# cloneofsimo/paint-with-words-sd

Hardware: NVIDIA H100
Metric: unet_steps_per_sec_512sq_cfg (higher is better)
Workload: dtype f16

## Files before the change

paint_with_words_sd_b200/csrc/attn_tc.cuh:

```cuda
#pragma once
#include "mma_sm90.cuh"
#include "pww_common.cuh"
#include "xattn_core.cuh"

namespace pww {
namespace fa {

constexpr int kThreads = core::kThreads;
constexpr int kBM = core::kBM;
constexpr int kBN = 64;

template <int D>
struct Cfg {
  using T_ = core::Tile<D>;
  static constexpr uint32_t KVBYTES = kBN * T_::LD * 2;
  static constexpr uint32_t OFF_KV = T_::QBYTES;
  static constexpr uint32_t SMEM = T_::QBYTES + 2 * 2 * KVBYTES;
  static_assert(SMEM <= 232448, "shared memory budget");
};

template <typename E>
struct Params {
  const E* q;
  const E* k;
  const E* v;
  E* out;
  int B, H, N;
  int64_t bs, rs;
  int64_t o_bs, o_rs;
  float scale;
};

template <int D, typename E>
constexpr int kMinBlocks = (D == 80 && std::is_same_v<E, __nv_bfloat16>) ? 1 : 0;

template <int D, typename E>
__global__ void __launch_bounds__(kThreads, kMinBlocks<D, E>) attn_fwd_kernel(const Params<E> p) {
  using C = core::Tile<D>;
  using CF = Cfg<D>;
  extern __shared__ __align__(128) unsigned char smem[];
  const uint32_t smem0 = ptx::smem_u32(smem);
  const int warp = threadIdx.x >> 5, lane = threadIdx.x & 31;
  const int qtiles = (p.N + kBM - 1) / kBM;
  const int bh = blockIdx.x / qtiles, qt = blockIdx.x - bh * qtiles;
  const int b = bh / p.H, h = bh - b * p.H;
  const int row_base = qt * kBM;
  const E* qb = p.q + (int64_t)b * p.bs + h * D;
  const E* kb = p.k + (int64_t)b * p.bs + h * D;
  const E* vb = p.v + (int64_t)b * p.bs + h * D;
  const int ntiles = (p.N + kBN - 1) / kBN;
  auto issue_kv = [&](int j) {
    const uint32_t st = smem0 + CF::OFF_KV + (j & 1) * 2 * CF::KVBYTES;
    const int rows = p.N - j * kBN < kBN ? p.N - j * kBN : kBN;
    core::load_rows<D>(st, kb + (int64_t)j * kBN * p.rs, p.rs, kBN, rows);
    core::load_rows<D>(st + CF::KVBYTES, vb + (int64_t)j * kBN * p.rs, p.rs, kBN, rows);
    ptx::cp_async_commit();
  };
  {
    const int rows = p.N - row_base < kBM ? p.N - row_base : kBM;
    core::load_rows<D>(smem0, qb + (int64_t)row_base * p.rs, p.rs, kBM, rows);
  }
  issue_kv(0);
  uint32_t qa[C::KS][4];
  float o[C::NT][4], m0, m1, l0, l1;
  core::warp_online_begin<D>(o, m0, m1, l0, l1);
  const float sl2 = p.scale * 1.4426950408889634f;
  const uint32_t qs = smem0 + (uint32_t)(warp * 16 * C::LD) * 2u;
#pragma unroll 1
  for (int jt = 0; jt < ntiles; ++jt) {
    if (jt + 1 < ntiles) {
      issue_kv(jt + 1);
      ptx::cp_async_wait<1>();
    } else {
      ptx::cp_async_wait<0>();
    }
    __syncthreads();
    if (jt == 0) {
#pragma unroll
      for (int kk = 0; kk < C::KS; ++kk)
        ptx::ldsm_x4(qs + (uint32_t)((lane & 15) * C::LD + kk * 16 + (lane >> 4) * 8) * 2u, qa[kk][0], qa[kk][1], qa[kk][2], qa[kk][3]);
    }
    const uint32_t ks = smem0 + CF::OFF_KV + (jt & 1) * 2 * CF::KVBYTES, vs = ks + CF::KVBYTES;
    float s[kBN / 8][4];
#pragma unroll
    for (int j = 0; j < kBN / 8; ++j) s[j][0] = s[j][1] = s[j][2] = s[j][3] = 0.f;
#pragma unroll
    for (int kk = 0; kk < C::KS; ++kk) {
#pragma unroll
      for (int jp = 0; jp < kBN / 16; ++jp) {
        const int t = 16 * jp + (lane & 7) + ((lane >> 4) << 3), d = kk * 16 + ((lane >> 3) & 1) * 8;
        uint32_t b0, b1, b2, b3;
        ptx::ldsm_x4(ks + (uint32_t)(t * C::LD + d) * 2u, b0, b1, b2, b3);
        ptx::mma16816<E>(s[2 * jp], qa[kk], b0, b1);
        ptx::mma16816<E>(s[2 * jp + 1], qa[kk], b2, b3);
      }
    }
    core::warp_online_chunk<D, E>(s, p.N - jt * kBN, sl2, vs, lane, o, m0, m1, l0, l1);
    __syncthreads();
  }
  core::warp_online_end<D>(o, l0, l1);
  core::warp_store<D>(o, smem + warp * 16 * C::LD * 2, lane, p.out + (int64_t)b * p.o_bs + h * D, p.o_rs,
                      row_base + warp * 16, p.N);
}

template <int D, typename E>
cudaError_t launch(const void* q, const void* k, const void* v, void* out, int B, int H, int N, int64_t bs, int64_t rs,
                   int64_t o_bs, int64_t o_rs, float scale, cudaStream_t s) {
  using CF = Cfg<D>;
  Params<E> p;
  p.q = (const E*)q; p.k = (const E*)k; p.v = (const E*)v; p.out = (E*)out;
  p.B = B; p.H = H; p.N = N; p.bs = bs; p.rs = rs; p.o_bs = o_bs; p.o_rs = o_rs; p.scale = scale;
  const cudaError_t e = allow_dynamic_smem<attn_fwd_kernel<D, E>>(CF::SMEM);
  if (e != cudaSuccess) return e;
  const long long grid = (long long)B * H * ((N + kBM - 1) / kBM);
  if (grid > 0x7fffffffLL) return cudaErrorInvalidConfiguration;
  attn_fwd_kernel<D, E><<<(unsigned)grid, kThreads, CF::SMEM, s>>>(p);
  return cudaGetLastError();
}

}
}
```

paint_with_words_sd_b200/csrc/pww_abi.cu:

```cuda
#include <stdio.h>
#include <string.h>

#include "pww_common.cuh"
#include "xattn_tc.cuh"
#include "xattn_fused2.cuh"
#include "attn_tc.cuh"
#include "unet_ops.cuh"
#include "sampler_step.cuh"
#include "control_inject.cuh"
#include "control_combine.cuh"
#include "adapter_residual.cuh"
#include <stdlib.h>
#include <algorithm>
#include <type_traits>

namespace {

thread_local char g_last_cuda_error[640] = "";

int cuda_fail(cudaError_t e);

bool aligned16(const void* p) { return (reinterpret_cast<uintptr_t>(p) & 15u) == 0; }

bool supported_head_dim(int D) { return D == 40 || D == 64 || D == 80 || D == 160; }

int check_common(const void* q, const void* k, int B, int H, int N, int T, int D, int64_t q_bs, int64_t q_rs,
                 int64_t k_bs, int64_t k_rs) {
  if (!q || !k || B <= 0 || H <= 0 || N <= 0 || T <= 0 || D <= 0) return PWW_ERR_BAD_ARG;
  if (!aligned16(q) || !aligned16(k)) return PWW_ERR_BAD_ARG;
  if ((q_bs | q_rs | k_bs | k_rs) & 7) return PWW_ERR_BAD_ARG;
  if (q_rs < (int64_t)H * D || k_rs < (int64_t)H * D) return PWW_ERR_BAD_ARG;
  if (!supported_head_dim(D) || !pww::core::supported_keys(T)) return PWW_ERR_UNSUPPORTED;
  return PWW_OK;
}

template <int D_, int KC_>
struct Shape {
  static constexpr int D = D_, KC = KC_;
};
template <int D, typename F>
cudaError_t with_chunks(int T, F&& f) {
  switch (pww::core::chunks_of(T)) {
    case 1: return f(Shape<D, 1>{});
    case 2: return f(Shape<D, 2>{});
    case 3: return f(Shape<D, 3>{});
  }
  return cudaErrorInvalidValue;
}
template <typename F>
cudaError_t with_shape(int D, int T, F&& f) {
  switch (D) {
    case 40: return with_chunks<40>(T, f);
    case 64: return with_chunks<64>(T, f);
    case 80: return with_chunks<80>(T, f);
    case 160: return with_chunks<160>(T, f);
  }
  return cudaErrorInvalidValue;
}

template <int lo, int hi, typename F>
void with_int(int v, F&& f) {
  if constexpr (lo < hi)
    if (v != lo) return with_int<lo + 1, hi>(v, f);
  f(std::integral_constant<int, lo>{});
}

size_t align_up(size_t x, size_t a) { return (x + a - 1) / a * a; }

constexpr int kStatSlotsPerImage = 2048;

int cuda_fail(cudaError_t e) {
  snprintf(g_last_cuda_error, sizeof(g_last_cuda_error), "%s: %s ", cudaGetErrorName(e), cudaGetErrorString(e));
  return PWW_ERR_CUDA;
}

template <typename E>
pww::XattnParams<E> xattn_params(const void* q, const void* k, const void* v, void* out, int B, int H, int N, int T, int D,
                                 int64_t q_bs, int64_t q_rs, int64_t k_bs, int64_t k_rs, int64_t o_bs, int64_t o_rs) {
  pww::XattnParams<E> p;
  memset(&p, 0, sizeof(p));
  p.q = (const E*)q; p.k = (const E*)k; p.v = (const E*)v; p.out = (E*)out;
  p.B = B; p.H = H; p.N = N; p.T = T; p.D = D;
  p.q_bs = q_bs; p.q_rs = q_rs; p.k_bs = k_bs; p.k_rs = k_rs; p.o_bs = o_bs; p.o_rs = o_rs;
  return p;
}

template <typename E>
pww::XattnParams<E> images(const pww::XattnParams<E>& p, int b0, int n) {
  pww::XattnParams<E> c = p;
  c.B = n;
  c.q += (int64_t)b0 * p.q_bs;
  c.k += (int64_t)b0 * p.k_bs;
  if (c.v) c.v += (int64_t)b0 * p.k_bs;
  if (c.out) c.out += (int64_t)b0 * p.o_bs;
  if (c.wmap_index) c.wmap_index += b0;
  if (c.stat_kind) c.stat_kind += b0;
  if (c.stats) c.stats += b0;
  if (c.stats_out) c.stats_out += b0;
  if (c.g_sigma) c.g_sigma += (int64_t)b0 * p.g_stride;
  return c;
}

}

extern "C" {

int pww_version(void) { return 300; }

const char* pww_status_str(int status) {
  switch (status) {
    case PWW_OK: return "ok";
    case PWW_ERR_BAD_ARG: return "bad argument (null/misaligned pointer, non-positive size or stride not a multiple of 8)";
    case PWW_ERR_UNSUPPORTED: return "unsupported shape or dtype (head dim must be 40/64/80/160, T <= 80, 154 or 231)";
    case PWW_ERR_CUDA: return "CUDA error (see pww_last_cuda_error)";
    case PWW_ERR_WORKSPACE: return "workspace too small (see pww_xattn_workspace_bytes)";
    default: return "unknown status";
  }
}

const char* pww_last_cuda_error(void) { return g_last_cuda_error; }

int pww_device_supported(void) {
  int dev = 0, major = 0;
  cudaError_t e = cudaGetDevice(&dev);
  if (e != cudaSuccess) return cuda_fail(e);
  e = cudaDeviceGetAttribute(&major, cudaDevAttrComputeCapabilityMajor, dev);
  if (e != cudaSuccess) return cuda_fail(e);
  return major == 9 ? 1 : 0;
}

size_t pww_xattn_workspace_bytes(int B, int H, int N, int T, int D) {
  (void)T; (void)D;
  if (B <= 0 || H <= 0 || N <= 0) return 0;
  return align_up((size_t)B * sizeof(unsigned int), 256) +
         (size_t)B * kStatSlotsPerImage * sizeof(pww::StatPartial);
}

}

namespace {

template <typename E>
int xattn_stats(const void* q, const void* k, int B, int H, int N, int T, int D, int64_t q_batch_stride,
                int64_t q_row_stride, int64_t k_batch_stride, int64_t k_row_stride, int stat, const int32_t* kinds,
                bool per_image, const int32_t* wmap_index, float* stats, void* workspace, size_t workspace_bytes,
                void* stream) {
  int rc = check_common(q, k, B, H, N, T, D, q_batch_stride, q_row_stride, k_batch_stride, k_row_stride);
  if (rc) return rc;
  if (!stats || !workspace) return PWW_ERR_BAD_ARG;
  if (per_image ? !kinds : (stat != PWW_STAT_MAX && stat != PWW_STAT_STD)) return PWW_ERR_BAD_ARG;
  if (workspace_bytes < pww_xattn_workspace_bytes(B, H, N, T, D)) return PWW_ERR_WORKSPACE;
  if (pww::num_sms() > kStatSlotsPerImage) return PWW_ERR_WORKSPACE;
  pww::XattnParams<E> p = xattn_params<E>(q, k, nullptr, nullptr, B, H, N, T, D, q_batch_stride, q_row_stride,
                                          k_batch_stride, k_row_stride, 0, 0);
  p.wmap_index = wmap_index; p.stat = stat; p.stat_kind = per_image ? kinds : nullptr; p.stats_out = stats;
  p.counters = (unsigned int*)workspace;
  p.partials = (pww::StatPartial*)((char*)workspace + align_up((size_t)B * sizeof(unsigned int), 256));
  for (int b0 = 0; b0 < B; b0 += pww::tc::kMaxBatch) {
    const pww::XattnParams<E> c = images(p, b0, std::min(B - b0, pww::tc::kMaxBatch));
    const cudaError_t e =
        with_shape(D, T, [&](auto k) { return pww::tc::launch_stats<k.D, k.KC>(c, (cudaStream_t)stream); });
    if (e != cudaSuccess) return cuda_fail(e);
  }
  return PWW_OK;
}

template <typename E>
int xattn_fwd(const void* q, const void* k, const void* v, void* out, int B, int H, int N, int T, int D,
              int64_t q_batch_stride, int64_t q_row_stride, int64_t k_batch_stride, int64_t k_row_stride,
              int64_t o_batch_stride, int64_t o_row_stride, const float* wmap, int64_t wmap_batch_stride,
              const int32_t* wmap_index, const float* stats, const float* g_sigma, int64_t g_stride, float scale,
              void* stream) {
  int rc = check_common(q, k, B, H, N, T, D, q_batch_stride, q_row_stride, k_batch_stride, k_row_stride);
  if (rc) return rc;
  if (!v || !out || !aligned16(v) || !aligned16(out)) return PWW_ERR_BAD_ARG;
  if ((o_batch_stride | o_row_stride) & 7 || o_row_stride < (int64_t)H * D) return PWW_ERR_BAD_ARG;
  if (wmap && (!stats || !g_sigma)) return PWW_ERR_BAD_ARG;
  pww::XattnParams<E> p = xattn_params<E>(q, k, v, out, B, H, N, T, D, q_batch_stride, q_row_stride, k_batch_stride,
                                          k_row_stride, o_batch_stride, o_row_stride);
  p.wmap = wmap; p.wmap_bs = wmap_batch_stride; p.wmap_index = wmap ? wmap_index : nullptr;
  p.stats = stats; p.g_sigma = g_sigma; p.g_stride = g_stride; p.scale = scale;
  for (int b0 = 0; b0 < B; b0 += pww::tc::kMaxBatch) {
    pww::XattnParams<E> c = images(p, b0, std::min(B - b0, pww::tc::kMaxBatch));
    if (wmap && !wmap_index) c.wmap += (int64_t)b0 * wmap_batch_stride;
    const cudaError_t e =
        with_shape(D, T, [&](auto k) { return pww::tc::launch_fwd<k.D, k.KC>(c, (cudaStream_t)stream); });
    if (e != cudaSuccess) return cuda_fail(e);
  }
  return PWW_OK;
}

template <typename E>
int xattn_fused(const void* q, const void* k, const void* v, void* out, int B, int H, int N, int T, int D,
                int64_t q_batch_stride, int64_t q_row_stride, int64_t k_batch_stride, int64_t k_row_stride,
                int64_t o_batch_stride, int64_t o_row_stride, const void* mpack, int64_t mpack_batch_stride, int Bw,
                const int8_t* cidx, const int32_t* wmap_index, int stat, const int32_t* kinds, bool per_image,
                const float* g_sigma, float scale, float* stats, void* workspace, size_t workspace_bytes,
                void* stream, const pww::fx::FxRecord* rec = nullptr) {
  int rc = check_common(q, k, B, H, N, T, D, q_batch_stride, q_row_stride, k_batch_stride, k_row_stride);
  if (rc) return rc;
  if (!v || !out || !aligned16(v) || !aligned16(out)) return PWW_ERR_BAD_ARG;
  if ((o_batch_stride | o_row_stride) & 7 || o_row_stride < (int64_t)H * D || o_batch_stride <= 0) return PWW_ERR_BAD_ARG;
  if (rec && (!rec->ridx || !rec->rec_index || !rec->rec_acc || !aligned16(rec->rec_acc) ||
              rec->rec_bs < (int64_t)H * N * pww::core::kRegions))
    return PWW_ERR_BAD_ARG;
  if (mpack) {
    if (!cidx || !g_sigma || !workspace || Bw <= 0 || !aligned16(mpack)) return PWW_ERR_BAD_ARG;
    if ((mpack_batch_stride & 7) || mpack_batch_stride < (int64_t)N * pww::fx::kMW) return PWW_ERR_BAD_ARG;
    if (per_image ? !kinds : (stat != PWW_STAT_MAX && stat != PWW_STAT_STD)) return PWW_ERR_BAD_ARG;
    if (workspace_bytes < pww_xattn_fused_workspace_bytes()) return PWW_ERR_WORKSPACE;
  }
  pww::XattnParams<E> p = xattn_params<E>(q, k, v, out, B, H, N, T, D, q_batch_stride, q_row_stride, k_batch_stride,
                                          k_row_stride, o_batch_stride, o_row_stride);
  p.g_sigma = g_sigma; p.g_stride = per_image ? 1 : 0; p.scale = scale; p.stat = stat;
  p.stat_kind = per_image ? kinds : nullptr; p.stats_out = stats;
  p.wmap_index = mpack ? wmap_index : nullptr;
  p.counters = (unsigned int*)workspace;
  p.partials = workspace ? (pww::StatPartial*)((char*)workspace + 512) : nullptr;
  int chunk = pww::fx::kMaxBatch;
  const int tiles = pww::ceil_div(N, pww::core::kBM);
  const int hg = pww::ceil_div(H, D == 40 ? pww::fx::Cfg2<40>::G : (D == 64 ? pww::fx::Cfg2<64>::G : 1));
  while (chunk > 1) {
    const int cb = B < chunk ? B : chunk;
    if (pww::fx::fused2_fits(cb, hg, tiles, pww::fx::fused_grid(cb * hg * tiles))) break;
    chunk >>= 1;
  }
  for (int b0 = 0; b0 < B; b0 += chunk) {
    pww::XattnParams<E> c = images(p, b0, std::min(B - b0, chunk));
    const void* mp = mpack;
    const int8_t* ci = cidx;
    if (mpack && !wmap_index) {
      mp = (const __half*)mpack + (int64_t)b0 * mpack_batch_stride;
      ci = cidx + (int64_t)b0 * pww::core::kTP * pww::core::chunks_of(T);
    }
    c.wmap = (const float*)mp;
    pww::fx::FxRecord r;
    if (rec) {
      r = *rec;
      r.rec_index += b0;
    }
    const cudaError_t e = with_shape(D, T, [&](auto k) {
      return pww::fx::launch_fused2<k.D, k.KC>(c, mp, mpack_batch_stride, ci, (cudaStream_t)stream, rec ? &r : nullptr);
    });
    if (e == cudaErrorInvalidConfiguration) return PWW_ERR_UNSUPPORTED;
    if (e != cudaSuccess) return cuda_fail(e);
  }
  return PWW_OK;
}

template <typename E>
int groupnorm_nhwc(const void* x, const void* add, int64_t add_batch_stride, const void* gamma, const void* beta, void* y,
                   int B, int HW, int C, int G, float eps, int silu, void* workspace, size_t workspace_bytes,
                   void* stream) {
  if (!x || !gamma || !beta || !y || !workspace || B <= 0 || HW <= 0 || C <= 0 || G <= 0) return PWW_ERR_BAD_ARG;
  if (!aligned16(x) || !aligned16(y) || !aligned16(gamma) || !aligned16(beta) || (add && !aligned16(add)))
    return PWW_ERR_BAD_ARG;
  if ((C & 7) || (C % G) || G > 64 || (C >> 3) > 1024) return PWW_ERR_UNSUPPORTED;
  if (add && ((add_batch_stride & 7) || add_batch_stride < C)) return PWW_ERR_BAD_ARG;
  if (workspace_bytes < pww_groupnorm_workspace_bytes(B, HW, G)) return PWW_ERR_WORKSPACE;
  const pww::uops::GnSplit sp = pww::uops::gn_split(HW, C, G);
  pww::uops::GnParams<E> p;
  p.x = (const E*)x; p.add = (const E*)add; p.add_bs = add_batch_stride; p.gamma = (const E*)gamma; p.beta = (const E*)beta;
  p.y = (E*)y;
  p.partial = (float2*)workspace;
  p.HW = HW; p.C = C; p.G = G; p.eps = eps; p.silu = silu;
  p.sv = sp.sv; p.chunks = sp.chunks; p.rows_per_chunk = sp.rows_per_chunk;
  cudaStream_t s = (cudaStream_t)stream;
  const size_t smem1 = (64 + (size_t)2 * sp.rpp * sp.sv * 8) * sizeof(float);
  if (smem1 > 48 * 1024) {
    const cudaError_t e = pww::allow_dynamic_smem<pww::uops::gn_stats_kernel<E>>(64 * 1024 + 256);
    if (e != cudaSuccess) return cuda_fail(e);
  }
  pww::uops::gn_stats_kernel<E><<<dim3(sp.chunks, sp.slices, B), sp.threads, smem1, s>>>(p);
  int rows = 4;
  while (rows > 1 && (long long)B * sp.slices * pww::ceil_div(HW, sp.rpp * rows) < 2 * pww::num_sms()) rows >>= 1;
  cudaLaunchAttribute pdl;
  pdl.id = cudaLaunchAttributeProgrammaticStreamSerialization;
  pdl.val.programmaticStreamSerializationAllowed = 1;
  cudaLaunchConfig_t cfg = {};
  cfg.gridDim = dim3(pww::ceil_div(HW, sp.rpp * rows), sp.slices, B);
  cfg.blockDim = dim3(sp.threads);
  cfg.stream = s;
  cfg.attrs = &pdl;
  cfg.numAttrs = 1;
  cudaError_t e = cudaLaunchKernelEx(&cfg, pww::uops::gn_apply_kernel<E>, p, sp.rpp * rows);
  if (e == cudaSuccess) e = cudaGetLastError();
  return e == cudaSuccess ? PWW_OK : cuda_fail(e);
}

template <typename E>
int geglu(const void* in, void* out, int64_t M, int I, void* stream) {
  if (!in || !out || M <= 0 || I <= 0 || !aligned16(in) || !aligned16(out)) return PWW_ERR_BAD_ARG;
  if (I & 7) return PWW_ERR_UNSUPPORTED;
  const long long total = (long long)M * (I >> 3);
  long long blocks = (total + 255) / 256;
  const long long cap = (long long)pww::num_sms() * 16;
  if (blocks > cap) blocks = cap;
  pww::uops::geglu_kernel<E><<<(int)blocks, 256, 0, (cudaStream_t)stream>>>((const E*)in, (E*)out, M, I);
  cudaError_t e = cudaGetLastError();
  return e == cudaSuccess ? PWW_OK : cuda_fail(e);
}

template <typename E>
int add_layernorm(const void* x, const void* res, const void* gamma, const void* beta, void* sum_out, void* y, int64_t M,
                  int C, float eps, void* stream) {
  if (!x || !gamma || !beta || !y || M <= 0 || C <= 0) return PWW_ERR_BAD_ARG;
  if (!aligned16(x) || !aligned16(y) || !aligned16(gamma) || !aligned16(beta) || (res && !aligned16(res)) ||
      (sum_out && !aligned16(sum_out)))
    return PWW_ERR_BAD_ARG;
  if ((C & 7) || C > 2048) return PWW_ERR_UNSUPPORTED;
  const int warps = 8;
  const unsigned grid = (unsigned)((M + warps - 1) / warps);
  with_int<1, 8>(((C >> 3) + 31) / 32, [&](auto vpl) {
    pww::uops::add_layernorm_kernel<E, vpl><<<grid, warps * 32, 0, (cudaStream_t)stream>>>(
        (const E*)x, (const E*)res, (const E*)gamma, (const E*)beta, (E*)sum_out, (E*)y, M, C, eps);
  });
  cudaError_t e = cudaGetLastError();
  return e == cudaSuccess ? PWW_OK : cuda_fail(e);
}

template <typename E>
int resnet_residual(const void* a, const void* h, const float* bias, void* out, int64_t rows, int C, void* stream) {
  if (!a || !h || !bias || !out || rows <= 0 || C <= 0 || (C & 7)) return PWW_ERR_BAD_ARG;
  if (!aligned16(a) || !aligned16(h) || !aligned16(bias) || !aligned16(out)) return PWW_ERR_BAD_ARG;
  const long long total = (long long)rows * (C >> 3);
  long long blocks = (total + 255) / 256;
  const long long cap = (long long)pww::num_sms() * 16;
  if (blocks > cap) blocks = cap;
  pww::uops::resnet_residual_kernel<E><<<(int)blocks, 256, 0, (cudaStream_t)stream>>>(
      (const E*)a, (const E*)h, bias, (E*)out, total, C >> 3);
  cudaError_t e = cudaGetLastError();
  return e == cudaSuccess ? PWW_OK : cuda_fail(e);
}

template <typename E>
int adapter_residual(const void* a, const void* b, const float* bias, const void* feat, void* out, int rows,
                     int64_t pixels, int C, int feat_rows, void* stream) {
  if (!a || !b || !out || rows <= 0 || pixels <= 0 || C <= 0 || (C & 7)) return PWW_ERR_BAD_ARG;
  if (feat_rows < 0 || feat_rows > rows || (feat_rows > 0 && !feat)) return PWW_ERR_BAD_ARG;
  if (!aligned16(a) || !aligned16(b) || !aligned16(out) || (bias && !aligned16(bias)) || (feat && !aligned16(feat)))
    return PWW_ERR_BAD_ARG;
  const long long per_row = (long long)pixels * (C >> 3);
  const cudaError_t e = pww::adp::launch<E>(a, b, bias, feat, out, (long long)rows * per_row,
                                            (long long)feat_rows * per_row, C >> 3, (long long)pww::num_sms() * 16,
                                            (cudaStream_t)stream);
  return e == cudaSuccess ? PWW_OK : cuda_fail(e);
}

template <typename E>
int attn_fwd(const void* q,const void* k, const void* v, void* out, int B, int H, int N, int D, int64_t qkv_batch_stride,
             int64_t qkv_row_stride, int64_t o_batch_stride, int64_t o_row_stride, float scale, void* stream) {
  if (!q || !k || !v || !out || B <= 0 || H <= 0 || N <= 0 || D <= 0) return PWW_ERR_BAD_ARG;
  if (!aligned16(q) || !aligned16(k) || !aligned16(v) || !aligned16(out)) return PWW_ERR_BAD_ARG;
  if ((qkv_batch_stride | qkv_row_stride | o_batch_stride | o_row_stride) & 7) return PWW_ERR_BAD_ARG;
  if (qkv_row_stride < (int64_t)H * D || o_row_stride < (int64_t)H * D) return PWW_ERR_BAD_ARG;
  if (!supported_head_dim(D)) return PWW_ERR_UNSUPPORTED;
  const cudaError_t e = with_shape(D, 1, [&](auto sh) {
    return pww::fa::launch<sh.D, E>(q, k, v, out, B, H, N, qkv_batch_stride, qkv_row_stride, o_batch_stride,
                                    o_row_stride, scale, (cudaStream_t)stream);
  });
  return e == cudaSuccess ? PWW_OK : cuda_fail(e);
}

template <typename E>
int control_inject(int n, void* const* dst, const void* const* res, const int64_t* elems_per_image, int rows,
                   const float* scales, void* stream) {
  if (n < 1 || n > pww::ctl::kMaxLevels || rows < 1 || !dst || !res || !elems_per_image) return PWW_ERR_BAD_ARG;
  pww::ctl::InjectArgs a;
  a.off[0] = 0;
  for (int k = 0; k < n; ++k) {
    const int64_t e = elems_per_image[k];
    if (e <= 0 || (e % pww::ctl::kVec) != 0) return PWW_ERR_BAD_ARG;
    if (!dst[k] || !res[k] || !aligned16(dst[k]) || !aligned16(res[k])) return PWW_ERR_BAD_ARG;
    a.dst[k] = dst[k];
    a.res[k] = res[k];
    a.vec_per_image[k] = e / pww::ctl::kVec;
    a.off[k + 1] = a.off[k] + (int64_t)rows * a.vec_per_image[k];
  }
  for (int k = n; k < pww::ctl::kMaxLevels; ++k) {
    a.dst[k] = nullptr;
    a.res[k] = nullptr;
    a.vec_per_image[k] = 0;
    a.off[k + 1] = a.off[n];
  }
  a.scales = scales;
  a.n = n;
  a.rows = rows;
  const cudaError_t e = pww::ctl::launch_inject<E>(a, (int64_t)pww::num_sms() * 8, (cudaStream_t)stream);
  return e == cudaSuccess ? PWW_OK : cuda_fail(e);
}

template <typename E>
int control_combine(int units, int n, void* const* out, const void* const* res, const int64_t* elems_per_image,
                    int rows, const float* scales, void* stream) {
  if (units < 1 || units > pww::ctl::kMaxUnits || n < 1 || n > pww::ctl::kMaxLevels || rows < 1 || !out || !res ||
      !elems_per_image || !scales)
    return PWW_ERR_BAD_ARG;
  pww::ctl::CombineArgs a = {};
  for (int k = 0; k < n; ++k) {
    const int64_t e = elems_per_image[k];
    if (e <= 0 || (e % pww::ctl::kVec) != 0) return PWW_ERR_BAD_ARG;
    if (!out[k] || !aligned16(out[k])) return PWW_ERR_BAD_ARG;
    a.out[k] = out[k];
    a.vec_per_image[k] = e / pww::ctl::kVec;
    a.off[k + 1] = a.off[k] + (int64_t)rows * a.vec_per_image[k];
  }
  for (int i = 0; i < units * n; ++i) {
    if (!res[i] || !aligned16(res[i])) return PWW_ERR_BAD_ARG;
    a.res[i] = res[i];
  }
  for (int k = n; k < pww::ctl::kMaxLevels; ++k) a.off[k + 1] = a.off[n];
  a.scales = scales;
  a.units = units;
  a.n = n;
  a.rows = rows;
  const cudaError_t e = pww::ctl::launch_combine<E>(a, (int64_t)pww::num_sms() * 8, (cudaStream_t)stream);
  return e == cudaSuccess ? PWW_OK : cuda_fail(e);
}

}

extern "C" {

int pww_xattn_stats_f16(const void* q, const void* k, int B, int H, int N, int T, int D, int64_t q_batch_stride,
    int64_t q_row_stride, int64_t k_batch_stride, int64_t k_row_stride, int stat, const int32_t* wmap_index,
    float* stats, void* workspace, size_t workspace_bytes, void* stream) {
  return xattn_stats<__half>(
      q, k, B, H, N, T, D, q_batch_stride, q_row_stride, k_batch_stride, k_row_stride, stat, nullptr, false,
      wmap_index, stats, workspace, workspace_bytes, stream);
}
int pww_xattn_stats_bf16(const void* q, const void* k, int B, int H, int N, int T, int D, int64_t q_batch_stride,
    int64_t q_row_stride, int64_t k_batch_stride, int64_t k_row_stride, int stat, const int32_t* wmap_index,
    float* stats, void* workspace, size_t workspace_bytes, void* stream) {
  return xattn_stats<__nv_bfloat16>(
      q, k, B, H, N, T, D, q_batch_stride, q_row_stride, k_batch_stride, k_row_stride, stat, nullptr, false,
      wmap_index, stats, workspace, workspace_bytes, stream);
}

int pww_xattn_stats_multi_f16(const void* q, const void* k, int B, int H, int N, int T, int D, int64_t q_batch_stride,
    int64_t q_row_stride, int64_t k_batch_stride, int64_t k_row_stride, const int32_t* stat, const int32_t* wmap_index,
    float* stats, void* workspace, size_t workspace_bytes, void* stream) {
  return xattn_stats<__half>(
      q, k, B, H, N, T, D, q_batch_stride, q_row_stride, k_batch_stride, k_row_stride, PWW_STAT_MAX, stat, true,
      wmap_index, stats, workspace, workspace_bytes, stream);
}
int pww_xattn_stats_multi_bf16(const void* q, const void* k, int B, int H, int N, int T, int D, int64_t q_batch_stride,
    int64_t q_row_stride, int64_t k_batch_stride, int64_t k_row_stride, const int32_t* stat, const int32_t* wmap_index,
    float* stats, void* workspace, size_t workspace_bytes, void* stream) {
  return xattn_stats<__nv_bfloat16>(
      q, k, B, H, N, T, D, q_batch_stride, q_row_stride, k_batch_stride, k_row_stride, PWW_STAT_MAX, stat, true,
      wmap_index, stats, workspace, workspace_bytes, stream);
}

int pww_xattn_fwd_f16(const void* q, const void* k, const void* v, void* out, int B, int H, int N, int T, int D,
    int64_t q_batch_stride, int64_t q_row_stride, int64_t k_batch_stride, int64_t k_row_stride, int64_t o_batch_stride,
    int64_t o_row_stride, const float* wmap, int64_t wmap_batch_stride, const int32_t* wmap_index, const float* stats,
    const float* g_sigma, float scale, void* stream) {
  return xattn_fwd<__half>(q, k, v, out, B, H, N, T, D, q_batch_stride, q_row_stride, k_batch_stride, k_row_stride,
      o_batch_stride, o_row_stride, wmap, wmap_batch_stride, wmap_index, stats, g_sigma, 0, scale, stream);
}
int pww_xattn_fwd_bf16(const void* q, const void* k, const void* v, void* out, int B, int H, int N, int T, int D,
    int64_t q_batch_stride, int64_t q_row_stride, int64_t k_batch_stride, int64_t k_row_stride, int64_t o_batch_stride,
    int64_t o_row_stride, const float* wmap, int64_t wmap_batch_stride, const int32_t* wmap_index, const float* stats,
    const float* g_sigma, float scale, void* stream) {
  return xattn_fwd<__nv_bfloat16>(
      q, k, v, out, B, H, N, T, D, q_batch_stride, q_row_stride, k_batch_stride, k_row_stride,
      o_batch_stride, o_row_stride, wmap, wmap_batch_stride, wmap_index, stats, g_sigma, 0, scale, stream);
}

int pww_xattn_fwd_multi_f16(const void* q, const void* k, const void* v, void* out, int B, int H, int N, int T, int D,
    int64_t q_batch_stride, int64_t q_row_stride, int64_t k_batch_stride, int64_t k_row_stride, int64_t o_batch_stride,
    int64_t o_row_stride, const float* wmap, int64_t wmap_batch_stride, const int32_t* wmap_index, const float* stats,
    const float* g_sigma, float scale, void* stream) {
  return xattn_fwd<__half>(q, k, v, out, B, H, N, T, D, q_batch_stride, q_row_stride, k_batch_stride, k_row_stride,
      o_batch_stride, o_row_stride, wmap, wmap_batch_stride, wmap_index, stats, g_sigma, 1, scale, stream);
}
int pww_xattn_fwd_multi_bf16(const void* q, const void* k, const void* v, void* out, int B, int H, int N, int T, int D,
    int64_t q_batch_stride, int64_t q_row_stride, int64_t k_batch_stride, int64_t k_row_stride, int64_t o_batch_stride,
    int64_t o_row_stride, const float* wmap, int64_t wmap_batch_stride, const int32_t* wmap_index, const float* stats,
    const float* g_sigma, float scale, void* stream) {
  return xattn_fwd<__nv_bfloat16>(
      q, k, v, out, B, H, N, T, D, q_batch_stride, q_row_stride, k_batch_stride, k_row_stride,
      o_batch_stride, o_row_stride, wmap, wmap_batch_stride, wmap_index, stats, g_sigma, 1, scale, stream);
}

size_t pww_xattn_fused_workspace_bytes(void) { return pww::fx::fused_workspace_bytes(); }

int pww_xattn_fused_f16(const void* q, const void* k, const void* v, void* out, int B, int H, int N, int T, int D,
    int64_t q_batch_stride, int64_t q_row_stride, int64_t k_batch_stride, int64_t k_row_stride, int64_t o_batch_stride,
    int64_t o_row_stride, const void* mpack, int64_t mpack_batch_stride, int Bw, const int8_t* cidx,
    const int32_t* wmap_index, int stat, const float* g_sigma, float scale, float* stats, void* workspace,
    size_t workspace_bytes, void* stream) {
  return xattn_fused<__half>(q, k, v, out, B, H, N, T, D, q_batch_stride, q_row_stride, k_batch_stride, k_row_stride,
      o_batch_stride, o_row_stride, mpack, mpack_batch_stride, Bw, cidx, wmap_index, stat, nullptr, false,
      g_sigma, scale, stats, workspace, workspace_bytes, stream);
}
int pww_xattn_fused_bf16(const void* q, const void* k, const void* v, void* out, int B, int H, int N, int T, int D,
    int64_t q_batch_stride, int64_t q_row_stride, int64_t k_batch_stride, int64_t k_row_stride, int64_t o_batch_stride,
    int64_t o_row_stride, const void* mpack, int64_t mpack_batch_stride, int Bw, const int8_t* cidx,
    const int32_t* wmap_index, int stat, const float* g_sigma, float scale, float* stats, void* workspace,
    size_t workspace_bytes, void* stream) {
  return xattn_fused<__nv_bfloat16>(
      q, k, v, out, B, H, N, T, D, q_batch_stride, q_row_stride, k_batch_stride, k_row_stride,
      o_batch_stride, o_row_stride, mpack, mpack_batch_stride, Bw, cidx, wmap_index, stat, nullptr, false,
      g_sigma, scale, stats, workspace, workspace_bytes, stream);
}

int pww_xattn_fused_multi_f16(const void* q, const void* k, const void* v, void* out, int B, int H, int N, int T, int D,
    int64_t q_batch_stride, int64_t q_row_stride, int64_t k_batch_stride, int64_t k_row_stride, int64_t o_batch_stride,
    int64_t o_row_stride, const void* mpack, int64_t mpack_batch_stride, int Bw, const int8_t* cidx,
    const int32_t* wmap_index, const int32_t* stat, const float* g_sigma, float scale, float* stats, void* workspace,
    size_t workspace_bytes, void* stream) {
  return xattn_fused<__half>(q, k, v, out, B, H, N, T, D, q_batch_stride, q_row_stride, k_batch_stride, k_row_stride,
      o_batch_stride, o_row_stride, mpack, mpack_batch_stride, Bw, cidx, wmap_index, PWW_STAT_MAX, stat, true,
      g_sigma, scale, stats, workspace, workspace_bytes, stream);
}
int pww_xattn_fused_multi_bf16(const void* q, const void* k, const void* v, void* out, int B, int H, int N, int T, int D,
    int64_t q_batch_stride, int64_t q_row_stride, int64_t k_batch_stride, int64_t k_row_stride, int64_t o_batch_stride,
    int64_t o_row_stride, const void* mpack, int64_t mpack_batch_stride, int Bw, const int8_t* cidx,
    const int32_t* wmap_index, const int32_t* stat, const float* g_sigma, float scale, float* stats, void* workspace,
    size_t workspace_bytes, void* stream) {
  return xattn_fused<__nv_bfloat16>(
      q, k, v, out, B, H, N, T, D, q_batch_stride, q_row_stride, k_batch_stride, k_row_stride,
      o_batch_stride, o_row_stride, mpack, mpack_batch_stride, Bw, cidx, wmap_index, PWW_STAT_MAX, stat, true,
      g_sigma, scale, stats, workspace, workspace_bytes, stream);
}

int pww_xattn_fused_rec_f16(const void* q, const void* k, const void* v, void* out, int B, int H, int N, int T, int D,
    int64_t q_batch_stride, int64_t q_row_stride, int64_t k_batch_stride, int64_t k_row_stride, int64_t o_batch_stride,
    int64_t o_row_stride, const void* mpack, int64_t mpack_batch_stride, int Bw, const int8_t* cidx,
    const int32_t* wmap_index, const int32_t* stat, const float* g_sigma, float scale, float* stats, void* workspace,
    size_t workspace_bytes, void* stream, const int8_t* ridx, const int32_t* rec_index, float* rec_acc,
    int64_t rec_batch_stride) {
  const pww::fx::FxRecord rec = {ridx, rec_index, rec_acc, rec_batch_stride};
  return xattn_fused<__half>(q, k, v, out, B, H, N, T, D, q_batch_stride, q_row_stride, k_batch_stride, k_row_stride,
      o_batch_stride, o_row_stride, mpack, mpack_batch_stride, Bw, cidx, wmap_index, PWW_STAT_MAX, stat, true,
      g_sigma, scale, stats, workspace, workspace_bytes, stream, &rec);
}
int pww_xattn_fused_rec_bf16(const void* q, const void* k, const void* v, void* out, int B, int H, int N, int T, int D,
    int64_t q_batch_stride, int64_t q_row_stride, int64_t k_batch_stride, int64_t k_row_stride, int64_t o_batch_stride,
    int64_t o_row_stride, const void* mpack, int64_t mpack_batch_stride, int Bw, const int8_t* cidx,
    const int32_t* wmap_index, const int32_t* stat, const float* g_sigma, float scale, float* stats, void* workspace,
    size_t workspace_bytes, void* stream, const int8_t* ridx, const int32_t* rec_index, float* rec_acc,
    int64_t rec_batch_stride) {
  const pww::fx::FxRecord rec = {ridx, rec_index, rec_acc, rec_batch_stride};
  return xattn_fused<__nv_bfloat16>(
      q, k, v, out, B, H, N, T, D, q_batch_stride, q_row_stride, k_batch_stride, k_row_stride,
      o_batch_stride, o_row_stride, mpack, mpack_batch_stride, Bw, cidx, wmap_index, PWW_STAT_MAX, stat, true,
      g_sigma, scale, stats, workspace, workspace_bytes, stream, &rec);
}

int pww_attn_fwd_f16(const void* q, const void* k, const void* v, void* out, int B, int H, int N, int D,
    int64_t qkv_batch_stride, int64_t qkv_row_stride, int64_t o_batch_stride, int64_t o_row_stride, float scale,
    void* stream) {
  return attn_fwd<__half>(
      q, k, v, out, B, H, N, D, qkv_batch_stride, qkv_row_stride, o_batch_stride, o_row_stride, scale, stream);
}
int pww_attn_fwd_bf16(const void* q, const void* k, const void* v, void* out, int B, int H, int N, int D,
    int64_t qkv_batch_stride, int64_t qkv_row_stride, int64_t o_batch_stride, int64_t o_row_stride, float scale,
    void* stream) {
  return attn_fwd<__nv_bfloat16>(
      q, k, v, out, B, H, N, D, qkv_batch_stride, qkv_row_stride, o_batch_stride, o_row_stride, scale, stream);
}

size_t pww_groupnorm_workspace_bytes(int B, int HW, int G) {
  if (B <= 0 || HW <= 0 || G <= 0) return 0;
  const size_t chunks = (size_t)std::min(HW, pww::uops::kGnMaxChunks);
  return align_up((size_t)B * G * chunks * sizeof(float2), 256);
}

int pww_groupnorm_nhwc_f16(const void* x, const void* add, int64_t add_batch_stride, const void* gamma,
    const void* beta, void* y, int B, int HW, int C, int G, float eps, int silu, void* workspace, size_t workspace_bytes,
    void* stream) {
  return groupnorm_nhwc<__half>(
      x, add, add_batch_stride, gamma, beta, y, B, HW, C, G, eps, silu, workspace, workspace_bytes,
      stream);
}
int pww_groupnorm_nhwc_bf16(const void* x, const void* add, int64_t add_batch_stride, const void* gamma,
    const void* beta, void* y, int B, int HW, int C, int G, float eps, int silu, void* workspace, size_t workspace_bytes,
    void* stream) {
  return groupnorm_nhwc<__nv_bfloat16>(
      x, add, add_batch_stride, gamma, beta, y, B, HW, C, G, eps, silu, workspace, workspace_bytes,
      stream);
}

int pww_geglu_f16(const void* in, void* out, int64_t M, int I, void* stream) {
  return geglu<__half>(in, out, M, I, stream);
}
int pww_geglu_bf16(const void* in, void* out, int64_t M, int I, void* stream) {
  return geglu<__nv_bfloat16>(in, out, M, I, stream);
}

int pww_add_layernorm_f16(const void* x, const void* res, const void* gamma, const void* beta, void* sum_out, void* y,
    int64_t M, int C, float eps, void* stream) {
  return add_layernorm<__half>(x, res, gamma, beta, sum_out, y, M, C, eps, stream);
}
int pww_add_layernorm_bf16(const void* x, const void* res, const void* gamma, const void* beta, void* sum_out, void* y,
    int64_t M, int C, float eps, void* stream) {
  return add_layernorm<__nv_bfloat16>(x, res, gamma, beta, sum_out, y, M, C, eps, stream);
}

int pww_resnet_residual_f16(const void* a, const void* h, const float* bias, void* out, int64_t rows, int C,
                            void* stream) {
  return resnet_residual<__half>(a, h, bias, out, rows, C, stream);
}
int pww_resnet_residual_bf16(const void* a, const void* h, const float* bias, void* out, int64_t rows, int C,
                             void* stream) {
  return resnet_residual<__nv_bfloat16>(a, h, bias, out, rows, C, stream);
}

int pww_adapter_residual_f16(const void* a, const void* b, const float* bias, const void* feat, void* out, int rows,
                             int64_t pixels, int C, int feat_rows, void* stream) {
  return adapter_residual<__half>(a, b, bias, feat, out, rows, pixels, C, feat_rows, stream);
}
int pww_adapter_residual_bf16(const void* a, const void* b, const float* bias, const void* feat, void* out, int rows,
                              int64_t pixels, int C, int feat_rows, void* stream) {
  return adapter_residual<__nv_bfloat16>(a, b, bias, feat, out, rows, pixels, C, feat_rows, stream);
}

int pww_sampler_input(const float* latents, const float* scale, const float* extra, void* out, int out_dtype, int m,
                      int channels, int height, int width, void* stream) {
  if (!latents || !scale || !out || m <= 0 || height <= 0 || width <= 0) return PWW_ERR_BAD_ARG;
  if (channels != 4 && channels != 9) return PWW_ERR_BAD_ARG;
  if ((channels == 9) != (extra != nullptr)) return PWW_ERR_BAD_ARG;
  if (out_dtype != PWW_DTYPE_F32 && out_dtype != PWW_DTYPE_F16 && out_dtype != PWW_DTYPE_BF16) return PWW_ERR_UNSUPPORTED;
  pww::smp::InputArgs a;
  a.lat = latents; a.scale = scale; a.extra = extra; a.out = out; a.m = m; a.C = channels; a.hw = height * width;
  const bool px4 = (a.hw % 4) == 0 && aligned16(latents) && (!extra || aligned16(extra)) && aligned16(out);
  cudaStream_t s = (cudaStream_t)stream;
  const cudaError_t e = out_dtype == PWW_DTYPE_F16    ? pww::smp::launch_input<__half>(a, px4, s)
                        : out_dtype == PWW_DTYPE_BF16 ? pww::smp::launch_input<__nv_bfloat16>(a, px4, s)
                                                      : pww::smp::launch_input<float>(a, px4, s);
  return e == cudaSuccess ? PWW_OK : cuda_fail(e);
}

int pww_sampler_update(const void* eps, int eps_dtype, int64_t eps_batch_stride, int64_t eps_channel_stride,
                       int64_t eps_row_stride, int64_t eps_col_stride, float* latents, float* history, int history_len,
                       const float* noise, const float* guidance, const float* beta, const float* form, int m,
                       int height, int width, void* stream) {
  if (!eps || !latents || !history || !guidance || !beta || !form) return PWW_ERR_BAD_ARG;
  if (m <= 0 || height <= 0 || width <= 0 || history_len < 1 || history_len > 4) return PWW_ERR_BAD_ARG;
  if (eps_dtype != PWW_DTYPE_F32 && eps_dtype != PWW_DTYPE_F16 && eps_dtype != PWW_DTYPE_BF16) return PWW_ERR_UNSUPPORTED;
  pww::smp::UpdateArgs a;
  a.eps = eps; a.e_sn = eps_batch_stride; a.e_sc = eps_channel_stride; a.e_sh = eps_row_stride; a.e_sw = eps_col_stride;
  a.lat = latents; a.hist = history; a.noise = noise; a.gscale = guidance; a.beta = beta; a.form = form;
  a.m = m; a.h = height; a.w = width; a.nh = history_len;
  const int64_t hw = (int64_t)height * width;
  const size_t es = eps_dtype == PWW_DTYPE_F32 ? 4 : 2;
  const bool px4 = (hw % 4) == 0 && aligned16(latents) && aligned16(history) && (!noise || aligned16(noise));
  const size_t need = px4 ? 16 : 4 * es;
  const bool cl = eps_channel_stride == 1 && eps_col_stride == 4 && eps_row_stride == 4 * (int64_t)width &&
                  (reinterpret_cast<uintptr_t>(eps) % need) == 0 && ((size_t)eps_batch_stride * es) % need == 0;
  cudaStream_t s = (cudaStream_t)stream;
  const cudaError_t e = eps_dtype == PWW_DTYPE_F16    ? pww::smp::launch_update<__half>(a, px4, cl, s)
                        : eps_dtype == PWW_DTYPE_BF16 ? pww::smp::launch_update<__nv_bfloat16>(a, px4, cl, s)
                                                      : pww::smp::launch_update<float>(a, px4, cl, s);
  return e == cudaSuccess ? PWW_OK : cuda_fail(e);
}

int pww_control_inject_f16(int n, void* const* dst, const void* const* res, const int64_t* elems_per_image, int rows,
                           const float* scales, void* stream) {
  return control_inject<__half>(n, dst, res, elems_per_image, rows, scales, stream);
}
int pww_control_inject_bf16(int n, void* const* dst, const void* const* res, const int64_t* elems_per_image, int rows,
                            const float* scales, void* stream) {
  return control_inject<__nv_bfloat16>(n, dst, res, elems_per_image, rows, scales, stream);
}

int pww_control_combine_f16(int units, int n, void* const* out, const void* const* res,
                            const int64_t* elems_per_image, int rows, const float* scales, void* stream) {
  return control_combine<__half>(units, n, out, res, elems_per_image, rows, scales, stream);
}
int pww_control_combine_bf16(int units, int n, void* const* out, const void* const* res,
                             const int64_t* elems_per_image, int rows, const float* scales, void* stream) {
  return control_combine<__nv_bfloat16>(units, n, out, res, elems_per_image, rows, scales, stream);
}

int pww_debug_fwd_schedule(int B, int H, int tiles, int grid, const int* wmap_index, int* out) {
  if (!wmap_index || !out) return PWW_ERR_BAD_ARG;
  return pww::tc::fwd_schedule_host(B, H, tiles, grid, wmap_index, out);
}

int pww_debug_set_fused_grid(int grid) {
  pww::fx::debug_grid() = grid < 0 ? 0 : grid;
  return PWW_OK;
}
int pww_debug_fused2_schedule(int B, int H, int G, int tiles, int grid, const int* wmap_index, int* out, int max_jobs) {
  if (!wmap_index || !out) return PWW_ERR_BAD_ARG;
  return pww::fx::fused2_schedule_host(B, H, G, tiles, grid, wmap_index, out, max_jobs);
}
int pww_debug_fused2_heads_per_unit(void) { return pww::fx::Cfg2<40>::G; }
int pww_debug_set_fused_jobs_dump(void* device_buffer) {
  pww::fx::debug_jobs_dump() = (unsigned*)device_buffer;
  return PWW_OK;
}
int pww_debug_fused_cta_has_image(int cta, int grid, int B, int H, int tiles, const int* wmap_index, int b) {
  if (!wmap_index) return PWW_ERR_BAD_ARG;
  return pww::fx::fused_cta_has_image_host(cta, grid, B, H, tiles, wmap_index, b);
}

}
```

Before: 159.9.

## Add cluster-based split-KV slicing and adaptive query-row tiles to self-attention

Self-attention CTAs can now split the key/value tiles across a thread-block cluster. Each CTA writes its partial output, max and sum into the owners' shared memory through distributed shared memory. The partials are then merged with a log-sum-exp combine. Query rows per CTA (64 or 128, with a matching warp count) are chosen from N to reduce padded rows, and launches go through cudaLaunchKernelEx with a cluster attribute. Slicing defaults to 1, so by default only the row-size choice and the new launch path change; the split path is meant for small grids and adds cluster syncs and merge work.

Result: no change. 159.6 (median of 6 runs) (-0.2%).

```diff
diff --git a/paint_with_words_sd_b200/csrc/attn_tc.cuh b/paint_with_words_sd_b200/csrc/attn_tc.cuh
--- a/paint_with_words_sd_b200/csrc/attn_tc.cuh
+++ b/paint_with_words_sd_b200/csrc/attn_tc.cuh
@@ -1,4 +1,6 @@
 #pragma once
+#include <cooperative_groups.h>
+
 #include "mma_sm90.cuh"
 #include "pww_common.cuh"
 #include "xattn_core.cuh"
@@ -6,18 +8,50 @@
 namespace pww {
 namespace fa {
 
-constexpr int kThreads = core::kThreads;
-constexpr int kBM = core::kBM;
 constexpr int kBN = 64;
-
-template <int D>
+constexpr int kMaxSlices = 8;
+
+template <int D, int W>
 struct Cfg {
   using T_ = core::Tile<D>;
+  static constexpr int R = 16 * W;
+  static constexpr uint32_t QBYTES = R * T_::LD * 2;
   static constexpr uint32_t KVBYTES = kBN * T_::LD * 2;
-  static constexpr uint32_t OFF_KV = T_::QBYTES;
-  static constexpr uint32_t SMEM = T_::QBYTES + 2 * 2 * KVBYTES;
+  static constexpr uint32_t OFF_KV = QBYTES;
+  static constexpr uint32_t SMEM = QBYTES + 2 * 2 * KVBYTES;
+  static constexpr int OLD = D + 4;
+  static_assert((R + kMaxSlices - 1) * (OLD + 2) * 4 <= SMEM, "slice partials fit in the dynamic shared memory");
   static_assert(SMEM <= 232448, "shared memory budget");
 };
+
+struct Plan {
+  int rows, slices, slice_tiles;
+};
+
+inline Plan make_plan(int N, int rows, int slices) {
+  const int tiles = ceil_div(N, kBN);
+  if (slices > tiles) slices = tiles;
+  const int st = ceil_div(tiles, slices);
+  return {rows, ceil_div(tiles, st), st};
+}
+
+inline int& debug_rows() {
+  static int r = 0;
+  return r;
+}
+inline int& debug_slices() {
+  static int s = 0;
+  return s;
+}
+
+inline Plan plan_for(int N, int D) {
+  (void)D;
+  const int rows = ceil_div(N, 64) < 2 * ceil_div(N, 128) ? 64 : 128;
+  Plan p = make_plan(N, rows, 1);
+  if (debug_rows() || debug_slices())
+    p = make_plan(N, debug_rows() ? debug_rows() : p.rows, debug_slices() ? debug_slices() : p.slices);
+  return p;
+}
 
 template <typename E>
 struct Params {
@@ -29,36 +63,42 @@
   int64_t bs, rs;
   int64_t o_bs, o_rs;
   float scale;
+  int slices, slice_tiles;
 };
 
-template <int D, typename E>
-constexpr int kMinBlocks = (D == 80 && std::is_same_v<E, __nv_bfloat16>) ? 1 : 0;
-
-template <int D, typename E>
-__global__ void __launch_bounds__(kThreads, kMinBlocks<D, E>) attn_fwd_kernel(const Params<E> p) {
+template <int D, typename E, int W>
+constexpr int kMinBlocks = std::is_same_v<E, __nv_bfloat16> && ((W == 8 && (D == 80 || D == 64)) || (W == 4 && D == 40))
+                               ? 1 : 0;
+
+template <int D, typename E, int W>
+__global__ void __launch_bounds__(W * 32, kMinBlocks<D, E, W>) attn_fwd_kernel(const Params<E> p) {
   using C = core::Tile<D>;
-  using CF = Cfg<D>;
+  using CF = Cfg<D, W>;
+  constexpr int R = CF::R;
   extern __shared__ __align__(128) unsigned char smem[];
   const uint32_t smem0 = ptx::smem_u32(smem);
   const int warp = threadIdx.x >> 5, lane = threadIdx.x & 31;
-  const int qtiles = (p.N + kBM - 1) / kBM;
-  const int bh = blockIdx.x / qtiles, qt = blockIdx.x - bh * qtiles;
+  const int qtiles = (p.N + R - 1) / R;
+  const int tile_id = blockIdx.x / p.slices, slice = blockIdx.x - tile_id * p.slices;
+  const int bh = tile_id / qtiles, qt = tile_id - bh * qtiles;
   const int b = bh / p.H, h = bh - b * p.H;
-  const int row_base = qt * kBM;
+  const int row_base = qt * R;
   const E* qb = p.q + (int64_t)b * p.bs + h * D;
   const E* kb = p.k + (int64_t)b * p.bs + h * D;
   const E* vb = p.v + (int64_t)b * p.bs + h * D;
-  const int ntiles = (p.N + kBN - 1) / kBN;
-  auto issue_kv = [&](int j) {
-    const uint32_t st = smem0 + CF::OFF_KV + (j & 1) * 2 * CF::KVBYTES;
+  const int t0 = slice * p.slice_tiles, all_tiles = (p.N + kBN - 1) / kBN;
+  const int ntiles = min(p.slice_tiles, all_tiles - t0);
+  auto issue_kv = [&](int jt) {
+    const uint32_t st = smem0 + CF::OFF_KV + (jt & 1) * 2 * CF::KVBYTES;
+    const int j = t0 + jt;
     const int rows = p.N - j * kBN < kBN ? p.N - j * kBN : kBN;
     core::load_rows<D>(st, kb + (int64_t)j * kBN * p.rs, p.rs, kBN, rows);
     core::load_rows<D>(st + CF::KVBYTES, vb + (int64_t)j * kBN * p.rs, p.rs, kBN, rows);
     ptx::cp_async_commit();
   };
   {
-    const int rows = p.N - row_base < kBM ? p.N - row_base : kBM;
-    core::load_rows<D>(smem0, qb + (int64_t)row_base * p.rs, p.rs, kBM, rows);
+    const int rows = p.N - row_base < R ? p.N - row_base : R;
+    core::load_rows<D>(smem0, qb + (int64_t)row_base * p.rs, p.rs, R, rows);
   }
   issue_kv(0);
   uint32_t qa[C::KS][4];
@@ -95,26 +135,107 @@
         ptx::mma16816<E>(s[2 * jp + 1], qa[kk], b2, b3);
       }
     }
-    core::warp_online_chunk<D, E>(s, p.N - jt * kBN, sl2, vs, lane, o, m0, m1, l0, l1);
+    core::warp_online_chunk<D, E>(s, p.N - (t0 + jt) * kBN, sl2, vs, lane, o, m0, m1, l0, l1);
     __syncthreads();
   }
-  core::warp_online_end<D>(o, l0, l1);
-  core::warp_store<D>(o, smem + warp * 16 * C::LD * 2, lane, p.out + (int64_t)b * p.o_bs + h * D, p.o_rs,
-                      row_base + warp * 16, p.N);
+  E* const ob = p.out + (int64_t)b * p.o_bs + h * D;
+  if (p.slices == 1) {
+    core::warp_online_end<D>(o, l0, l1);
+    core::warp_store<D>(o, smem + warp * 16 * C::LD * 2, lane, ob, p.o_rs, row_base + warp * 16, p.N);
+    return;
+  }
+
+  const int S = p.slices, share = (R + S - 1) / S;
+  float* const po = reinterpret_cast<float*>(smem);
+  float* const pm = po + S * share * CF::OLD;
+  float* const pl = pm + S * share;
+  l0 += __shfl_xor_sync(0xffffffffu, l0, 1);
+  l0 += __shfl_xor_sync(0xffffffffu, l0, 2);
+  l1 += __shfl_xor_sync(0xffffffffu, l1, 1);
+  l1 += __shfl_xor_sync(0xffffffffu, l1, 2);
+  cooperative_groups::cluster_group cluster = cooperative_groups::this_cluster();
+  cluster.sync();
+  {
+    const int g = lane >> 2, q = lane & 3;
+#pragma unroll
+    for (int hf = 0; hf < 2; ++hf) {
+      const int r = warp * 16 + g + 8 * hf, owner = r / share;
+      const int slot = slice * share + (r - owner * share);
+      float* const dst = cluster.map_shared_rank(po, owner) + slot * CF::OLD;
+#pragma unroll
+      for (int j = 0; j < C::NT; ++j)
+        *reinterpret_cast<float2*>(dst + 8 * j + 2 * q) = make_float2(o[j][2 * hf], o[j][2 * hf + 1]);
+      if (q == 0) {
+        *cluster.map_shared_rank(pm + slot, owner) = hf ? m1 : m0;
+        *cluster.map_shared_rank(pl + slot, owner) = hf ? l1 : l0;
+      }
+    }
+  }
+  cluster.sync();
+
+  const int r0 = slice * share, nr = min(share, R - r0);
+  constexpr int NC = D / 8;
+  for (int idx = threadIdx.x; idx < nr * NC; idx += W * 32) {
+    const int lr = idx / NC, c = idx - lr * NC;
+    if (row_base + r0 + lr >= p.N) continue;
+    float m = -INFINITY;
+    for (int s = 0; s < S; ++s) m = fmaxf(m, pm[s * share + lr]);
+    float l = 0.f, acc[8];
+#pragma unroll
+    for (int e = 0; e < 8; ++e) acc[e] = 0.f;
+    for (int s = 0; s < S; ++s) {
+      const float ms = pm[s * share + lr];
+      const float w = ms == -INFINITY ? 0.f : ptx::ex2((ms - m) * sl2);
+      l = fmaf(pl[s * share + lr], w, l);
+      const float4* src = reinterpret_cast<const float4*>(po + (s * share + lr) * CF::OLD + 8 * c);
+      const float4 x = src[0], y = src[1];
+      acc[0] = fmaf(x.x, w, acc[0]); acc[1] = fmaf(x.y, w, acc[1]);
+      acc[2] = fmaf(x.z, w, acc[2]); acc[3] = fmaf(x.w, w, acc[3]);
+      acc[4] = fmaf(y.x, w, acc[4]); acc[5] = fmaf(y.y, w, acc[5]);
+      acc[6] = fmaf(y.z, w, acc[6]); acc[7] = fmaf(y.w, w, acc[7]);
+    }
+    const float inv = 1.f / l;
+    uint4 pk;
+    pk.x = ptx::pack2<E>(acc[0] * inv, acc[1] * inv);
+    pk.y = ptx::pack2<E>(acc[2] * inv, acc[3] * inv);
+    pk.z = ptx::pack2<E>(acc[4] * inv, acc[5] * inv);
+    pk.w = ptx::pack2<E>(acc[6] * inv, acc[7] * inv);
+    *reinterpret_cast<uint4*>(ob + (int64_t)(row_base + r0 + lr) * p.o_rs + c * 8) = pk;
+  }
+}
+
+template <int D, typename E, int W>
+cudaError_t launch_rows(const Params<E>& p, int B, int H, int N, cudaStream_t s) {
+  using CF = Cfg<D, W>;
+  const cudaError_t e = allow_dynamic_smem<attn_fwd_kernel<D, E, W>>(CF::SMEM);
+  if (e != cudaSuccess) return e;
+  const long long grid = (long long)B * H * ((N + CF::R - 1) / CF::R) * p.slices;
+  if (grid > 0x7fffffffLL) return cudaErrorInvalidConfiguration;
+  cudaLaunchConfig_t cfg = {};
+  cfg.gridDim = dim3((unsigned)grid);
+  cfg.blockDim = dim3(W * 32);
+  cfg.dynamicSmemBytes = CF::SMEM;
+  cfg.stream = s;
+  cudaLaunchAttribute attr[1];
+  attr[0].id = cudaLaunchAttributeClusterDimension;
+  attr[0].val.clusterDim.x = (unsigned)p.slices;
+  attr[0].val.clusterDim.y = 1;
+  attr[0].val.clusterDim.z = 1;
+  cfg.attrs = attr;
+  cfg.numAttrs = 1;
+  return cudaLaunchKernelEx(&cfg, attn_fwd_kernel<D, E, W>, p);
 }
 
 template <int D, typename E>
 cudaError_t launch(const void* q, const void* k, const void* v, void* out, int B, int H, int N, int64_t bs, int64_t rs,
                    int64_t o_bs, int64_t o_rs, float scale, cudaStream_t s) {
-  using CF = Cfg<D>;
+  const Plan pl = plan_for(N, D);
   Params<E> p;
   p.q = (const E*)q; p.k = (const E*)k; p.v = (const E*)v; p.out = (E*)out;
   p.B = B; p.H = H; p.N = N; p.bs = bs; p.rs = rs; p.o_bs = o_bs; p.o_rs = o_rs; p.scale = scale;
-  const cudaError_t e = allow_dynamic_smem<attn_fwd_kernel<D, E>>(CF::SMEM);
+  p.slices = pl.slices; p.slice_tiles = pl.slice_tiles;
+  const cudaError_t e = pl.rows == 64 ? launch_rows<D, E, 4>(p, B, H, N, s) : launch_rows<D, E, 8>(p, B, H, N, s);
   if (e != cudaSuccess) return e;
-  const long long grid = (long long)B * H * ((N + kBM - 1) / kBM);
-  if (grid > 0x7fffffffLL) return cudaErrorInvalidConfiguration;
-  attn_fwd_kernel<D, E><<<(unsigned)grid, kThreads, CF::SMEM, s>>>(p);
   return cudaGetLastError();
 }
 
diff --git a/paint_with_words_sd_b200/csrc/pww_abi.cu b/paint_with_words_sd_b200/csrc/pww_abi.cu
--- a/paint_with_words_sd_b200/csrc/pww_abi.cu
+++ b/paint_with_words_sd_b200/csrc/pww_abi.cu
@@ -694,6 +694,23 @@
   pww::fx::debug_jobs_dump() = (unsigned*)device_buffer;
   return PWW_OK;
 }
+int pww_debug_attn_plan(int B, int H, int N, int D, int* out) {
+  if (!out || B <= 0 || H <= 0 || N <= 0) return PWW_ERR_BAD_ARG;
+  if (!supported_head_dim(D)) return PWW_ERR_UNSUPPORTED;
+  const pww::fa::Plan p = pww::fa::plan_for(N, D);
+  out[0] = p.rows;
+  out[1] = p.slices;
+  out[2] = p.slice_tiles * pww::fa::kBN;
+  const long long grid = (long long)B * H * pww::ceil_div(N, p.rows) * p.slices;
+  out[3] = grid > 0x7fffffffLL ? -1 : (int)grid;
+  return PWW_OK;
+}
+int pww_debug_set_attn_plan(int rows, int slices) {
+  if ((rows != 0 && rows != 64 && rows != 128) || slices < 0 || slices > pww::fa::kMaxSlices) return PWW_ERR_BAD_ARG;
+  pww::fa::debug_rows() = rows;
+  pww::fa::debug_slices() = slices;
+  return PWW_OK;
+}
 int pww_debug_fused_cta_has_image(int cta, int grid, int B, int H, int tiles, const int* wmap_index, int b) {
   if (!wmap_index) return PWW_ERR_BAD_ARG;
   return pww::fx::fused_cta_has_image_host(cta, grid, B, H, tiles, wmap_index, b);
```
